# shravan-d/SculptMate

Measured on AMD Instinct MI355X. Metric: meshes/sec + ms/image, TripoSR 256^3 grid, at 1/2/4/8 MI355X, higher is better.
Workload: dtype fp32-equivalent (bf16 3-limb split, 24 bits, fp32 accumulate) density MLP / f32 tables, SiLU, marching cubes / bf16 transformer [filtered grid: an fp16 one-product pass decides the SIGN away from the level, every value marching cubes reads carries the three-limb value: mesh bit-identical to the full

## Files before the change

### sculptmate_amd/csrc/gemm.hip

```cpp
#include <stdlib.h>

#include <mutex>
#include <type_traits>

#include "common.h"

namespace sculpt {

typedef __bf16 bf16x8_t __attribute__((ext_vector_type(8)));
typedef __attribute__((address_space(3))) void *lds_ptr_t;
typedef const __attribute__((address_space(1))) void *gbl_ptr_t;

static constexpr int BM_DEFAULT = 128;
#ifndef SCULPT_GEMM_READ_AHEAD
#define SCULPT_GEMM_READ_AHEAD 1
#endif
static constexpr int BK = 64;

__device__ __forceinline__ float erf_as(float x) {
    const float ax = fabsf(x);
    const float t = __builtin_amdgcn_rcpf(fmaf(0.3275911f, ax, 1.0f));
    float p = fmaf(1.061405429f, t, -1.453152027f);
    p = fmaf(p, t, 1.421413741f);
    p = fmaf(p, t, -0.284496736f);
    p = fmaf(p, t, 0.254829592f);
    const float e = __builtin_amdgcn_exp2f(-1.44269504088896340736f * ax * ax);
    const float r = 1.0f - p * t * e;
    return copysignf(r, x);
}
__device__ __forceinline__ float gelu_erf(float x) { return 0.5f * x * (1.0f + erf_as(x * 0.70710678118654752440f)); }

__device__ __forceinline__ int lds_off(int r, int c) { return r * 128 + ((c ^ ((r >> 1) & 7)) << 4); }

struct GemmArgs {
    const uint16_t *A; int lda;
    const uint16_t *W; int ldw;
    const float *bias;
    const float *residual; int ldr;
    float *out_f32; uint16_t *out_bf16; int ldo;
    uint16_t *out_t; int ldt;
    int M, N, K;
    int n_split;
    int n_major;
    int n_store;
    int cv_H, cv_W, cv_c64, cv_dil;
    const uint16_t *cv_zero;
    const float *ln_stats; int ln_slots;
    const float *ln_colsum;
    float ln_eps;
    float *stats_out;
    int stats_ld;
    const float *zeros;
    int gm;
    int m_store;
    int stage;
    unsigned long long *stamps;
};

#ifdef SCULPT_EXPERIMENTS
unsigned long long *g_gemm_stamps = nullptr;
extern "C" void sculpt_experiment_gemm_stamps(void *p) { g_gemm_stamps = static_cast<unsigned long long *>(p); }
#endif

__device__ __forceinline__ void gemm_tile_of(const GemmArgs &g, int lin, int gx, int gy, int &nt, int &mt) {
    const int tile = xcd_tile(lin, gx * gy);
    if (g.gm > 0) {
        const int per = g.gm * gx, grp = tile / per, first = grp * g.gm, within = tile - grp * per;
        const int gsz = min(g.gm, gy - first);
        nt = within / gsz;
        mt = first + (within - nt * gsz);
    } else {
        nt = g.n_major ? tile / gy : tile % gx;
        mt = g.n_major ? tile % gy : tile / gx;
    }
}

static constexpr int LN_SLOT = 64;

template <int EPI, int BW, int NW, bool CONV = false, int BM = BM_DEFAULT, int NWR = 2, bool KS = false>
__global__ __launch_bounds__(NW * 64) void gemm_bf16_kernel(GemmArgs g) {
    static_assert(NWR == 2 || (EPI == SCULPT_EPI_NONE && !CONV), "the 4 x 2 wave grid is for the plain / residual / LayerNorm-fold form");
    static_assert(!KS || (NWR == 2 && NW == 8 && EPI == SCULPT_EPI_NONE && !CONV), "the k-split pairs are for the 8-wave plain form");
    constexpr int WT = BW * 128;
    constexpr int AT = BM * 128;
    constexpr int NSTAGE = (BW == 64 || BM == 96) ? 3 : 2;
    constexpr int DIST = NSTAGE - 1;
    constexpr int XCH = NSTAGE * (WT + AT);
    __shared__ __attribute__((aligned(16))) unsigned char smem[XCH + 2 * BM * 8];
    const int tid = threadIdx.x, lane = tid & 63;
    const int wave = __builtin_amdgcn_readfirstlane(tid >> 6);
    constexpr int NWC = NW / NWR;
    constexpr int WPW = BW / NWR;
    constexpr int TJ = BM / 16 / NWC;
    const int wr = wave / NWC, wc = wave % NWC;
    constexpr int NOUT = (EPI == SCULPT_EPI_GEGLU) ? BW / 2 : BW;
    constexpr int TI = WPW / 16;
    int nt_, mt_;
    gemm_tile_of(g, blockIdx.y * gridDim.x + blockIdx.x, gridDim.x, gridDim.y, nt_, mt_);
    const int n0 = nt_ * NOUT, m0 = mt_ * BM;
    GEMM_STAMP(g, 0);

    const int srow = lane >> 3, sslot = lane & 7;
    constexpr int WI = BW / 8 / NW;
    constexpr int AG = BM / 8, AI = (AG + NW - 1) / NW, AFULL = AG - NW * (AI - 1);
    constexpr bool UNEVEN = AG % NW != 0;
    const int acnt = (!UNEVEN || wave < AFULL) ? AI : AI - 1;
    const int abase = (!UNEVEN || wave < AFULL) ? wave * AI : AFULL * AI + (wave - AFULL) * (AI - 1);
    const uint16_t *wsrc0, *wsrc1, *wsrc2, *wsrc3;
    const uint16_t *asrc0, *asrc1, *asrc2, *asrc3;
    unsigned amask0 = 0, amask1 = 0, amask2 = 0, amask3 = 0;
    const uint16_t *zsrc = CONV ? g.cv_zero + (sslot << 3) : nullptr;
    {
        auto wrow = [&](int j) -> int {
            if (EPI == SCULPT_EPI_GEGLU) {
                const int sub = j >> 4, within = j & 15;
                return ((sub & 1) ? g.N : 0) + n0 + (sub >> 1) * 16 + within;
            }
            return n0 + j;
        };
        auto wp = [&](int q) -> const uint16_t * {
            const int r = 8 * (wave * WI + q) + srow;
            return g.W + (long)wrow(r) * g.ldw + ((sslot ^ ((r >> 1) & 7)) << 3);
        };
        auto ap = [&](int q) -> const uint16_t * {
            const int r = 8 * (abase + q) + srow;
            const int m = min(m0 + r, g.M - 1);
            return g.A + (long)m * g.lda + ((sslot ^ ((r >> 1) & 7)) << 3);
        };
        auto am = [&](int q) -> unsigned {
            if (!CONV) return 0u;
            const int r = 8 * (abase + q) + srow;
            const int m = min(m0 + r, g.M - 1);
            const int x = m % g.cv_W, y = (m / g.cv_W) % g.cv_H;
            unsigned mask = 0;
#pragma unroll
            for (int t = 0; t < 9; ++t) {
                const int yy = y + (t / 3 - 1) * g.cv_dil, xx = x + (t % 3 - 1) * g.cv_dil;
                mask |= (yy >= 0 && yy < g.cv_H && xx >= 0 && xx < g.cv_W) ? (1u << t) : 0u;
            }
            return mask;
        };
        wsrc0 = wp(0); wsrc1 = wp(1 % WI); wsrc2 = wp(2 % WI); wsrc3 = wp(3 % WI);
        asrc0 = ap(0); asrc1 = ap(1 % AI); asrc2 = ap(2 % AI); asrc3 = ap(3 % AI);
        amask0 = am(0); amask1 = am(1 % AI); amask2 = am(2 % AI); amask3 = am(3 % AI);
    }
    const int wdst = (wave * WI) * 1024, adst = abase * 1024;

#define STAGE(buf, kt)                                                                                       \
    do {                                                                                                     \
        unsigned char *wb = smem + (buf) * (WT + AT);                                                        \
        unsigned char *ab = wb + WT;                                                                         \
        const int ko = (kt) * BK;                                                                            \
        __builtin_amdgcn_global_load_lds((gbl_ptr_t)(wsrc0 + ko), (lds_ptr_t)(wb + wdst), 16, 0, 0);         \
        if (WI >= 2)                                                                                         \
            __builtin_amdgcn_global_load_lds((gbl_ptr_t)(wsrc1 + ko), (lds_ptr_t)(wb + wdst + 1024), 16, 0, 0); \
        if (WI == 4) {                                                                                       \
            __builtin_amdgcn_global_load_lds((gbl_ptr_t)(wsrc2 + ko), (lds_ptr_t)(wb + wdst + 2048), 16, 0, 0); \
            __builtin_amdgcn_global_load_lds((gbl_ptr_t)(wsrc3 + ko), (lds_ptr_t)(wb + wdst + 3072), 16, 0, 0); \
        }                                                                                                    \
        long ao = ko;                                                                                        \
        int tap = 0;                                                                                         \
        if (CONV) {                                                                                          \
            tap = (kt) / g.cv_c64;                                                                           \
            const int cc = (kt) - tap * g.cv_c64, dy = tap / 3 - 1, dx = tap - (tap / 3) * 3 - 1;            \
            ao = ((long)(dy * g.cv_dil) * g.cv_W + dx * g.cv_dil) * g.lda + cc * 64;                         \
        }                                                                                                    \
        const uint16_t *a0 = (!CONV || ((amask0 >> tap) & 1u)) ? asrc0 + ao : zsrc;                          \
        const uint16_t *a1 = (!CONV || ((amask1 >> tap) & 1u)) ? asrc1 + ao : zsrc;                          \
        __builtin_amdgcn_global_load_lds((gbl_ptr_t)a0, (lds_ptr_t)(ab + adst), 16, 0, 0);                   \
        if (AI >= 2 && (!UNEVEN || acnt >= 2))                                                               \
            __builtin_amdgcn_global_load_lds((gbl_ptr_t)a1, (lds_ptr_t)(ab + adst + 1024), 16, 0, 0);        \
        if (AI >= 3) {                                                                                       \
            const uint16_t *a2 = (!CONV || ((amask2 >> tap) & 1u)) ? asrc2 + ao : zsrc;                      \
            __builtin_amdgcn_global_load_lds((gbl_ptr_t)a2, (lds_ptr_t)(ab + adst + 2048), 16, 0, 0);        \
        }                                                                                                    \
        if (AI == 4) {                                                                                       \
            const uint16_t *a3 = (!CONV || ((amask3 >> tap) & 1u)) ? asrc3 + ao : zsrc;                      \
            __builtin_amdgcn_global_load_lds((gbl_ptr_t)a3, (lds_ptr_t)(ab + adst + 3072), 16, 0, 0);        \
        }                                                                                                    \
    } while (0)

    f32x4 acc[TI][TJ];
#pragma unroll
    for (int i = 0; i < TI; ++i)
#pragma unroll
        for (int j = 0; j < TJ; ++j) acc[i][j] = f32x4{0.f, 0.f, 0.f, 0.f};
    f32x4 acc2[KS ? 2 * TI : 1][KS ? TJ : 1];
    if (KS) {
#pragma unroll
        for (int i = 0; i < 2 * TI; ++i)
#pragma unroll
            for (int j = 0; j < TJ; ++j) acc2[KS ? i : 0][KS ? j : 0] = f32x4{0.f, 0.f, 0.f, 0.f};
    }

    const int nk = g.K / BK;
    const int fr = lane & 15, fq = lane >> 4;
    int aoff[TI], boff[TJ];
#pragma unroll
    for (int i = 0; i < TI; ++i) aoff[i] = lds_off(wr * WPW + i * 16 + fr, fq);
    int aoff2[KS ? 2 * TI : 1];
    if (KS) {
#pragma unroll
        for (int i = 0; i < 2 * TI; ++i) aoff2[KS ? i : 0] = lds_off((i / TI) * WPW + (i % TI) * 16 + fr, fq) ^ (wr << 6);
    }
#pragma unroll
    for (int j = 0; j < TJ; ++j) boff[j] = lds_off(wc * (16 * TJ) + j * 16 + fr, fq);

    constexpr int MAXU = 4;
    float2 sv[TJ][MAXU];
    const bool ln_load = g.ln_stats && wr == 0;
    if (ln_load) {
#pragma unroll
        for (int j = 0; j < TJ; ++j) {
            const int m = min(m0 + wc * (16 * TJ) + j * 16 + fr, g.M - 1);
            const float2 *sp = reinterpret_cast<const float2 *>(g.ln_stats) + m;
#pragma unroll
            for (int u = 0; u < MAXU; ++u) sv[j][u] = sp[(long)min(fq + 4 * u, g.ln_slots - 1) * g.stats_ld];
        }
    }

    constexpr int LPT = WI + AI;
    STAGE(0, 0);
    if (DIST > 1 && nk > 1) STAGE(1, 1);
    for (int kt = 0; kt < nk; ++kt) {
        const int buf = kt % NSTAGE;
        if (DIST > 1 && kt + 1 < nk && !(kt == 0 && g.ln_stats)) {
            if (!UNEVEN || acnt == AI) asm volatile("s_waitcnt vmcnt(%0)" ::"n"(LPT) : "memory");
            else asm volatile("s_waitcnt vmcnt(%0)" ::"n"(LPT - 1) : "memory");
        } else {
            asm volatile("s_waitcnt vmcnt(0)" ::: "memory");
        }
        __builtin_amdgcn_s_barrier();
#ifdef SCULPT_EXPERIMENTS
        if (kt == 0) GEMM_STAMP(g, 1);
#endif
        if (kt + DIST < nk) STAGE((kt + DIST) % NSTAGE, kt + DIST);
        const unsigned char *wb = smem + buf * (WT + AT);
        const unsigned char *ab = wb + WT;
        if constexpr (KS) {
            bf16x8_t af[2 * TI], bfr[TJ];
#pragma unroll
            for (int i = 0; i < 2 * TI; ++i) af[i] = *reinterpret_cast<const bf16x8_t *>(wb + aoff2[i]);
#pragma unroll
            for (int j = 0; j < TJ; ++j) bfr[j] = *reinterpret_cast<const bf16x8_t *>(ab + (boff[j] ^ (wr << 6)));
#pragma unroll
            for (int i = 0; i < 2 * TI; ++i)
#pragma unroll
                for (int j = 0; j < TJ; ++j)
                    acc2[i][j] = __builtin_amdgcn_mfma_f32_16x16x32_bf16(af[i], bfr[j], acc2[i][j], 0, 0, 0);
            __builtin_amdgcn_sched_group_barrier(0x100, 2 * TI + TJ, 0);
            __builtin_amdgcn_sched_group_barrier(0x8, 2 * TI * TJ, 0);
        } else if ((NW == 8 || (NW == 4 && BM == 96)) && SCULPT_GEMM_READ_AHEAD) {
            bf16x8_t af[2][TI], bfr[2][TJ];
#pragma unroll
            for (int ks = 0; ks < 2; ++ks) {
#pragma unroll
                for (int i = 0; i < TI; ++i) af[ks][i] = *reinterpret_cast<const bf16x8_t *>(wb + (aoff[i] ^ (ks << 6)));
#pragma unroll
                for (int j = 0; j < TJ; ++j) bfr[ks][j] = *reinterpret_cast<const bf16x8_t *>(ab + (boff[j] ^ (ks << 6)));
            }
#pragma unroll
            for (int ks = 0; ks < 2; ++ks)
#pragma unroll
                for (int i = 0; i < TI; ++i)
#pragma unroll
                    for (int j = 0; j < TJ; ++j)
                        acc[i][j] = __builtin_amdgcn_mfma_f32_16x16x32_bf16(af[ks][i], bfr[ks][j], acc[i][j], 0, 0, 0);
            __builtin_amdgcn_sched_group_barrier(0x100, 2 * (TI + TJ), 0);
            __builtin_amdgcn_sched_group_barrier(0x8, 2 * TI * TJ, 0);
        } else {
#pragma unroll
        for (int ks = 0; ks < 2; ++ks) {
            bf16x8_t af[TI], bfr[TJ];
#pragma unroll
            for (int i = 0; i < TI; ++i) af[i] = *reinterpret_cast<const bf16x8_t *>(wb + (aoff[i] ^ (ks << 6)));
#pragma unroll
            for (int j = 0; j < TJ; ++j) bfr[j] = *reinterpret_cast<const bf16x8_t *>(ab + (boff[j] ^ (ks << 6)));
#pragma unroll
            for (int i = 0; i < TI; ++i)
#pragma unroll
                for (int j = 0; j < TJ; ++j)
                    acc[i][j] = __builtin_amdgcn_mfma_f32_16x16x32_bf16(af[i], bfr[j], acc[i][j], 0, 0, 0);
        }
        }
    }
#undef STAGE
    if constexpr (KS) {
        asm volatile("s_waitcnt lgkmcnt(0)" ::: "memory");
        __builtin_amdgcn_s_barrier();
        f32x4 *xb = reinterpret_cast<f32x4 *>(smem);
        const int partner = (1 - wr) * NWC + wc;
        static_assert(NW * TI * TJ * 64 * 16 <= NSTAGE * (WT + AT), "the exchange fits the ring");
        if (wr == 0) {
#pragma unroll
            for (int i = 0; i < TI; ++i)
#pragma unroll
                for (int j = 0; j < TJ; ++j) xb[(wave * TI * TJ + i * TJ + j) * 64 + lane] = acc2[TI + i][j];
        } else {
#pragma unroll
            for (int i = 0; i < TI; ++i)
#pragma unroll
                for (int j = 0; j < TJ; ++j) xb[(wave * TI * TJ + i * TJ + j) * 64 + lane] = acc2[i][j];
        }
        asm volatile("s_waitcnt lgkmcnt(0)" ::: "memory");
        __builtin_amdgcn_s_barrier();
        if (wr == 0) {
#pragma unroll
            for (int i = 0; i < TI; ++i)
#pragma unroll
                for (int j = 0; j < TJ; ++j) acc[i][j] = acc2[i][j] + xb[(partner * TI * TJ + i * TJ + j) * 64 + lane];
        } else {
#pragma unroll
            for (int i = 0; i < TI; ++i)
#pragma unroll
                for (int j = 0; j < TJ; ++j) acc[i][j] = xb[(partner * TI * TJ + i * TJ + j) * 64 + lane] + acc2[TI + i][j];
        }
    }

    GEMM_STAMP(g, 2);
    float ln_mean[TJ], ln_rstd[TJ];
#pragma unroll
    for (int j = 0; j < TJ; ++j) { ln_mean[j] = 0.f; ln_rstd[j] = 1.f; }
    float2 *xch = reinterpret_cast<float2 *>(smem + XCH);
    if (g.ln_stats) {
        if (ln_load) {
            const float inv_slots = 1.0f / (float)g.ln_slots;
#pragma unroll
            for (int j = 0; j < TJ; ++j) {
                float sm = 0.f;
#pragma unroll
                for (int u = 0; u < MAXU; ++u) sm += (fq + 4 * u < g.ln_slots) ? sv[j][u].x : 0.f;
                sm += __shfl_xor(sm, 16, 64);
                sm += __shfl_xor(sm, 32, 64);
                const float mean = sm * inv_slots;
                float m2 = 0.f;
#pragma unroll
                for (int u = 0; u < MAXU; ++u) {
                    const float d = sv[j][u].x - mean;
                    m2 += (fq + 4 * u < g.ln_slots) ? fmaf((float)LN_SLOT * d, d, sv[j][u].y) : 0.f;
                }
                m2 += __shfl_xor(m2, 16, 64);
                m2 += __shfl_xor(m2, 32, 64);
                ln_mean[j] = mean;
                ln_rstd[j] = rsqrtf(m2 * inv_slots * (1.0f / LN_SLOT) + g.ln_eps);
                if (fq == 0) xch[wc * (16 * TJ) + j * 16 + fr] = make_float2(ln_mean[j], ln_rstd[j]);
            }
        }
        asm volatile("s_waitcnt lgkmcnt(0)" ::: "memory");
        __builtin_amdgcn_s_barrier();
        if (!ln_load) {
#pragma unroll
            for (int j = 0; j < TJ; ++j) {
                const float2 v = xch[wc * (16 * TJ) + j * 16 + fr];
                ln_mean[j] = v.x;
                ln_rstd[j] = v.y;
            }
        }
    }

    const float *biasp = g.bias ? g.bias : g.zeros;
    const float *csp = g.ln_stats ? g.ln_colsum : g.zeros;
    float4 b4[TI], c4[TI];
#pragma unroll
    for (int i = 0; i < TI; ++i) {
        const int wrow = (EPI == SCULPT_EPI_GEGLU) ? ((i & 1) ? g.N : 0) + n0 + (wr * (TI / 2) + (i >> 1)) * 16 + fq * 4
                                                   : n0 + wr * WPW + i * 16 + fq * 4;
        b4[i] = *reinterpret_cast<const float4 *>(biasp + wrow);
        c4[i] = *reinterpret_cast<const float4 *>(csp + wrow);
    }
    auto f4 = [](const float4 &v, int r) -> float { return r == 0 ? v.x : (r == 1 ? v.y : (r == 2 ? v.z : v.w)); };
    float4 rs[TI][TJ];
    if (EPI != SCULPT_EPI_GEGLU && g.residual) {
#pragma unroll
        for (int j = 0; j < TJ; ++j) {
            const int m = min(m0 + wc * (16 * TJ) + j * 16 + fr, g.M - 1);
#pragma unroll
            for (int i = 0; i < TI; ++i)
                rs[i][j] = *reinterpret_cast<const float4 *>(g.residual + (long)m * g.ldr + n0 + wr * WPW + i * 16 + fq * 4);
        }
    }
#pragma unroll
    for (int j = 0; j < TJ; ++j) {
        if (EPI == SCULPT_EPI_GEGLU) {
#pragma unroll
            for (int ip = 0; ip < TI / 2; ++ip)
#pragma unroll
                for (int r = 0; r < 4; ++r) {
                    const float v = ln_rstd[j] * (acc[2 * ip][j][r] - ln_mean[j] * f4(c4[2 * ip], r)) + f4(b4[2 * ip], r);
                    const float gt = ln_rstd[j] * (acc[2 * ip + 1][j][r] - ln_mean[j] * f4(c4[2 * ip + 1], r)) + f4(b4[2 * ip + 1], r);
                    acc[2 * ip][j][r] = v * gelu_erf(gt);
                }
        } else {
#pragma unroll
            for (int i = 0; i < TI; ++i)
#pragma unroll
                for (int r = 0; r < 4; ++r) {
                    float v = ln_rstd[j] * (acc[i][j][r] - ln_mean[j] * f4(c4[i], r)) + f4(b4[i], r);
                    if (EPI == SCULPT_EPI_GELU) v = gelu_erf(v);
                    if (EPI == SCULPT_EPI_RELU) v = fmaxf(v, 0.f);
                    if (g.residual) v += f4(rs[i][j], r);
                    acc[i][j][r] = v;
                }
        }
    }
    GEMM_STAMP(g, 3);
#pragma unroll
    for (int j = 0; j < TJ; ++j) {
        const int m = m0 + wc * (16 * TJ) + j * 16 + fr;
        if (m >= g.m_store) continue;
        if (EPI == SCULPT_EPI_GEGLU) {
#pragma unroll
            for (int ip = 0; ip < TI / 2; ++ip) {
                const int n = n0 + (wr * (TI / 2) + ip) * 16 + fq * 4;
                const f32x4 o = acc[2 * ip][j];
                if (g.out_bf16) {
                    uint2 pk;
                    pk.x = pack_bf16x2(o[0], o[1]);
                    pk.y = pack_bf16x2(o[2], o[3]);
                    *reinterpret_cast<uint2 *>(g.out_bf16 + (long)m * g.ldo + n) = pk;
                }
                if (g.out_f32) *reinterpret_cast<float4 *>(g.out_f32 + (long)m * g.ldo + n) = make_float4(o[0], o[1], o[2], o[3]);
            }
        } else {
#pragma unroll
            for (int i = 0; i < TI; ++i) {
                const int n = n0 + wr * WPW + i * 16 + fq * 4;
                if (n >= g.n_store) continue;
                const f32x4 o = acc[i][j];
                const bool tpart = n >= g.n_split;
                if (!tpart) {
                    if (g.out_f32) *reinterpret_cast<float4 *>(g.out_f32 + (long)m * g.ldo + n) = make_float4(o[0], o[1], o[2], o[3]);
                    if (g.out_bf16) {
                        uint2 pk;
                        pk.x = pack_bf16x2(o[0], o[1]);
                        pk.y = pack_bf16x2(o[2], o[3]);
                        *reinterpret_cast<uint2 *>(g.out_bf16 + (long)m * g.ldo + n) = pk;
                    }
                }
                if (g.out_t && (tpart || g.n_split >= g.N)) {
                    const int nt0 = tpart ? n - g.n_split : n;
#pragma unroll
                    for (int r = 0; r < 4; ++r) g.out_t[(long)(nt0 + r) * g.ldt + m] = f32_to_bf16(o[r]);
                }
            }
        }
    }
    if (EPI == SCULPT_EPI_NONE && g.stats_out) {
        constexpr int WCOLS = WPW;
        float pm[TJ], pq[TJ];
#pragma unroll
        for (int j = 0; j < TJ; ++j) {
            float sm = 0.f;
#pragma unroll
            for (int i = 0; i < TI; ++i) sm += (acc[i][j][0] + acc[i][j][1]) + (acc[i][j][2] + acc[i][j][3]);
            sm += __shfl_xor(sm, 16, 64);
            sm += __shfl_xor(sm, 32, 64);
            const float mean = sm * (1.0f / WCOLS);
            float m2 = 0.f;
#pragma unroll
            for (int i = 0; i < TI; ++i)
#pragma unroll
                for (int r = 0; r < 4; ++r) { const float d = acc[i][j][r] - mean; m2 = fmaf(d, d, m2); }
            m2 += __shfl_xor(m2, 16, 64);
            m2 += __shfl_xor(m2, 32, 64);
            pm[j] = mean;
            pq[j] = m2;
        }
        float2 *so = reinterpret_cast<float2 *>(g.stats_out);
        if (WCOLS == LN_SLOT) {
#pragma unroll
            for (int j = 0; j < TJ; ++j) {
                const int m = m0 + wc * (16 * TJ) + j * 16 + fr;
                if (fq == 0 && m < g.m_store) so[(long)((n0 + wr * WCOLS) / LN_SLOT) * g.stats_ld + m] = make_float2(pm[j], pq[j]);
            }
        } else {
            static_assert(WCOLS == LN_SLOT || 2 * WCOLS == LN_SLOT, "statistics slice = one or two waves' columns");
            if ((wr & 1) == 1 && fq == 0) {
#pragma unroll
                for (int j = 0; j < TJ; ++j) xch[(wr >> 1) * BM + wc * (16 * TJ) + j * 16 + fr] = make_float2(pm[j], pq[j]);
            }
            asm volatile("s_waitcnt lgkmcnt(0)" ::: "memory");
            __builtin_amdgcn_s_barrier();
            if ((wr & 1) == 0 && fq == 0) {
#pragma unroll
                for (int j = 0; j < TJ; ++j) {
                    const int m = m0 + wc * (16 * TJ) + j * 16 + fr;
                    const float2 o = xch[(wr >> 1) * BM + wc * (16 * TJ) + j * 16 + fr];
                    const float d = pm[j] - o.x;
                    if (m < g.m_store) so[(long)((n0 + wr * WCOLS) / LN_SLOT) * g.stats_ld + m] = make_float2(0.5f * (pm[j] + o.x), pq[j] + o.y + (0.5f * WCOLS) * d * d);
                }
            }
        }
    }
    GEMM_STAMP(g, 4);
    GEMM_STAMP_IDS(g);
}

template <int EPI, int BM, bool RES = false>
__global__ __launch_bounds__(512) void gemm256_kernel(GemmArgs g) {
    static_assert(BM == 256 || BM == 192, "activation rows per tile");
    static_assert(!RES || (BM == 192 && EPI == SCULPT_EPI_NONE), "the residual form: 192-row tiles, no activation");
    constexpr int BW = 256, NW = 8, NWC = 4, TI = 8, TJ = BM / 64, WROWS = BM / 4;
    constexpr int JB1 = TJ - 2, AU = BM / 64;
    constexpr int NU = 4 + AU;
    constexpr int WT = BW * 128, AT = BM * 128;
    constexpr int XCH = 2 * (WT + AT);
    constexpr int XBC = XCH + 2 * BM * 8;
    __shared__ __attribute__((aligned(16))) unsigned char smem[XBC + 2048];
    const int tid = threadIdx.x, lane = tid & 63;
    const int wave = __builtin_amdgcn_readfirstlane(tid >> 6);
    const int wr = wave / NWC, wc = wave % NWC;
    constexpr int NOUT = (EPI == SCULPT_EPI_GEGLU) ? BW / 2 : BW;
    int nt_, mt_;
    gemm_tile_of(g, blockIdx.y * gridDim.x + blockIdx.x, gridDim.x, gridDim.y, nt_, mt_);
    const int n0 = nt_ * NOUT, m0 = mt_ * BM;
    GEMM_STAMP(g, 0);

    const int srow = lane >> 3, sslot = lane & 7;
    unsigned woff[4], aof[4];
#pragma unroll
    for (int q = 0; q < 4; ++q) {
        const int r = 8 * (wave * 4 + q) + srow;
        const int ra = 8 * (wave * AU + (q < AU ? q : AU - 1)) + srow;
        int wrow = n0 + r;
        if (EPI == SCULPT_EPI_GEGLU) {
            const int sub = r >> 4, within = r & 15;
            wrow = ((sub & 1) ? g.N : 0) + n0 + (sub >> 1) * 16 + within;
        }
        woff[q] = ((unsigned)wrow * (unsigned)g.ldw + ((sslot ^ ((r >> 1) & 7)) << 3)) * 2u;
        aof[q] = ((unsigned)min(m0 + ra, g.M - 1) * (unsigned)g.lda + ((sslot ^ ((ra >> 1) & 7)) << 3)) * 2u;
    }
    const char *Wb = reinterpret_cast<const char *>(g.W), *Ab = reinterpret_cast<const char *>(g.A);
    const int sdst = wave * 4096, sdsta = wave * (AU * 1024);
#define G256_STAGE(buf, kt, u)                                                                                                   \
    do {                                                                                                                         \
        unsigned char *tb = smem + (buf) * (WT + AT) + ((u) >= 4 ? WT + sdsta : sdst) + ((u) & 3) * 1024;                        \
        const char *src = ((u) >= 4 ? Ab + aof[(u) & 3] : Wb + woff[(u) & 3]) + (size_t)(kt) * (BK * 2);                         \
        __builtin_amdgcn_global_load_lds((gbl_ptr_t)src, (lds_ptr_t)tb, 16, 0, 0);                                               \
    } while (0)

    const int nk = g.K / BK;
#pragma unroll
    for (int u = 0; u < NU; ++u) G256_STAGE(0, 0, u);
    if (nk > 1) {
#pragma unroll
        for (int u = 0; u < 6; ++u) G256_STAGE(1, 1, u);
    }

    const int fr = lane & 15, fq = lane >> 4;
    if (tid < 128) {
        const float *srcv = tid < 64 ? (g.bias ? g.bias : g.zeros) : (g.ln_stats ? g.ln_colsum : g.zeros);
        const int e = (tid & 63) * 4;
        const int row = EPI == SCULPT_EPI_GEGLU ? (e < 128 ? n0 + e : g.N + n0 + e - 128) : n0 + e;
        *reinterpret_cast<float4 *>(smem + XBC + (tid >> 6) * 1024 + e * 4) = *reinterpret_cast<const float4 *>(srcv + row);
    }
    float ln_mean[TJ], ln_rstd[TJ];
#pragma unroll
    for (int j = 0; j < TJ; ++j) { ln_mean[j] = 0.f; ln_rstd[j] = 1.f; }
    float2 *xch = reinterpret_cast<float2 *>(smem + XCH);
    if (g.ln_stats) {
        if (wr == 0) {
            constexpr int MAXU = 4;
            const float inv_slots = 1.0f / (float)g.ln_slots;
#pragma unroll
            for (int j = 0; j < TJ; ++j) {
                const int m = min(m0 + wc * WROWS + j * 16 + fr, g.M - 1);
                const float2 *sp = reinterpret_cast<const float2 *>(g.ln_stats) + m;
                float2 sv[MAXU];
#pragma unroll
                for (int u = 0; u < MAXU; ++u) sv[u] = sp[(long)min(fq + 4 * u, g.ln_slots - 1) * g.stats_ld];
                float sm = 0.f;
#pragma unroll
                for (int u = 0; u < MAXU; ++u) sm += (fq + 4 * u < g.ln_slots) ? sv[u].x : 0.f;
                sm += __shfl_xor(sm, 16, 64);
                sm += __shfl_xor(sm, 32, 64);
                const float mean = sm * inv_slots;
                float m2 = 0.f;
#pragma unroll
                for (int u = 0; u < MAXU; ++u) {
                    const float d = sv[u].x - mean;
                    m2 += (fq + 4 * u < g.ln_slots) ? fmaf((float)LN_SLOT * d, d, sv[u].y) : 0.f;
                }
                m2 += __shfl_xor(m2, 16, 64);
                m2 += __shfl_xor(m2, 32, 64);
                ln_mean[j] = mean;
                ln_rstd[j] = rsqrtf(m2 * inv_slots * (1.0f / LN_SLOT) + g.ln_eps);
                if (fq == 0) xch[wc * WROWS + j * 16 + fr] = make_float2(ln_mean[j], ln_rstd[j]);
            }
        }
        asm volatile("s_waitcnt lgkmcnt(0)" ::: "memory");
        __builtin_amdgcn_s_barrier();
        if (wr == 1) {
#pragma unroll
            for (int j = 0; j < TJ; ++j) {
                const float2 v = xch[wc * WROWS + j * 16 + fr];
                ln_mean[j] = v.x;
                ln_rstd[j] = v.y;
            }
        }
    }

    f32x4 acc[TI][TJ];
#pragma unroll
    for (int i = 0; i < TI; ++i)
#pragma unroll
        for (int j = 0; j < TJ; ++j) acc[i][j] = f32x4{0.f, 0.f, 0.f, 0.f};

    int aoff[4], boff[2];
#pragma unroll
    for (int i = 0; i < 4; ++i) aoff[i] = lds_off(wr * 128 + i * 16 + fr, fq);
#pragma unroll
    for (int j = 0; j < 2; ++j) boff[j] = WT + lds_off(wc * WROWS + j * 16 + fr, fq);
    bf16x8_t af[4][2], bq[4][2];
#define G256_LDA(buf, ih, i, ks) af[i][ks] = *reinterpret_cast<const bf16x8_t *>(smem + (buf) * (WT + AT) + (ih) * 8192 + (aoff[i] ^ ((ks) << 6)))
#define G256_LDB(buf, jh, j, ks) bq[2 * (jh) + (j)][ks] = *reinterpret_cast<const bf16x8_t *>(smem + (buf) * (WT + AT) + (jh) * 4096 + (boff[j] ^ ((ks) << 6)))
#define G256_MF(ih, jh, i, j, ks) \
    acc[4 * (ih) + (i)][2 * (jh) + (j)] = __builtin_amdgcn_mfma_f32_16x16x32_bf16(af[i][ks], bq[2 * (jh) + (j)][ks], acc[4 * (ih) + (i)][2 * (jh) + (j)], 0, 0, 0)
#define G256_FENCE __builtin_amdgcn_sched_barrier(0)

    if (nk > 1) asm volatile("s_waitcnt vmcnt(6)" ::: "memory");
    else asm volatile("s_waitcnt vmcnt(0)" ::: "memory");
    __builtin_amdgcn_s_barrier();
    GEMM_STAMP(g, 1);
#pragma unroll
    for (int ks = 0; ks < 2; ++ks) {
#pragma unroll
        for (int i = 0; i < 4; ++i) G256_LDA(0, 0, i, ks);
#pragma unroll
        for (int j = 0; j < 2; ++j) G256_LDB(0, 0, j, ks);
    }

    auto ktile = [&](int kt, auto more1_t, auto more2_t) __attribute__((always_inline)) {
        constexpr bool MORE1 = decltype(more1_t)::value, MORE2 = decltype(more2_t)::value;
        const int buf = kt & 1, nbuf = buf ^ 1;
#pragma unroll
        for (int ks = 0; ks < 2; ++ks)
#pragma unroll
            for (int i = 0; i < 4; ++i) {
                G256_MF(0, 0, i, 0, ks);
                G256_MF(0, 0, i, 1, ks);
                if (i < JB1) G256_LDB(buf, 1, i, ks);
                if (ks == 0 && i >= 2 && 4 + i < NU && MORE1) G256_STAGE(nbuf, kt + 1, 4 + i);
                G256_FENCE;
            }
#pragma unroll
        for (int ks = 0; ks < 2; ++ks)
#pragma unroll
            for (int i = 0; i < 4; ++i) {
                G256_MF(0, 1, i, 0, ks);
                if (JB1 == 2) G256_MF(0, 1, i, 1, ks);
                G256_LDA(buf, 1, i, ks);
                G256_FENCE;
            }
        asm volatile("s_waitcnt lgkmcnt(0)" ::: "memory");
        __builtin_amdgcn_s_barrier();
#pragma unroll
        for (int ks = 0; ks < 2; ++ks)
#pragma unroll
            for (int i = 0; i < 4; ++i) {
                G256_MF(1, 1, i, 0, ks);
                if (JB1 == 2) G256_MF(1, 1, i, 1, ks);
                if (ks == 0 && i < 3 && MORE2) G256_STAGE(buf, kt + 2, i);
                G256_FENCE;
            }
        if (MORE2) asm volatile("s_waitcnt vmcnt(3)" ::: "memory");
        else asm volatile("s_waitcnt vmcnt(0)" ::: "memory");
        __builtin_amdgcn_s_barrier();
#pragma unroll
        for (int ks = 0; ks < 2; ++ks)
#pragma unroll
            for (int i = 0; i < 4; ++i) {
                G256_MF(1, 0, i, 0, ks);
                G256_MF(1, 0, i, 1, ks);
                if (MORE1) G256_LDA(nbuf, 0, i, ks);
                if (MORE1 && i == 3) {
                    G256_LDB(nbuf, 0, 0, ks);
                    G256_LDB(nbuf, 0, 1, ks);
                }
                if (ks == 0 && i < 3 && MORE2) G256_STAGE(buf, kt + 2, 3 + i);
                G256_FENCE;
            }
    };
    {
// ... 503 lines not shown
```

Baseline: 124.5.

## Prefetch GEMM epilogue bias, colsum and residual loads inside the K loop

Splits the GEMM K loop into three modes so that the epilogue's bias/colsum and residual global loads are issued a few K-tiles before the end, behind the last stage prefetch. The vmcnt waits are adjusted to count these extra outstanding loads, which hides epilogue load latency under the final MFMA tiles. In exchange it raises register pressure by keeping the residual/bias registers live across the loop, and it relies on tricky vmcnt accounting.

```diff
diff --git a/sculptmate_amd/csrc/gemm.hip b/sculptmate_amd/csrc/gemm.hip
--- a/sculptmate_amd/csrc/gemm.hip
+++ b/sculptmate_amd/csrc/gemm.hip
@@ -14,6 +14,9 @@
 static constexpr int BM_DEFAULT = 128;
 #ifndef SCULPT_GEMM_READ_AHEAD
 #define SCULPT_GEMM_READ_AHEAD 1
+#endif
+#ifndef SCULPT_GEMM_EPI_AHEAD
+#define SCULPT_GEMM_EPI_AHEAD 1
 #endif
 static constexpr int BK = 64;
 
@@ -220,21 +223,85 @@
     }
 
     constexpr int LPT = WI + AI;
+
+    constexpr bool EPF = BW == 64, EPF_COL = EPF && BM != 64;
+    constexpr int EAHEAD = SCULPT_GEMM_EPI_AHEAD < DIST ? SCULPT_GEMM_EPI_AHEAD : DIST;
+    constexpr int EL_COL = EPF_COL ? 2 * TI : 0, EL_RES = (EPF && EPI != SCULPT_EPI_GEGLU) ? TI * TJ : 0;
+    static_assert(LPT + EL_COL + EL_RES <= 63, "vmcnt is a 6-bit counter");
+    static_assert(EAHEAD >= 1 && EAHEAD <= DIST, "every wait behind the prefetch is for a K-tile older than the epilogue loads");
+    const bool has_res = EPI != SCULPT_EPI_GEGLU && g.residual;
+    const float *biasp = g.bias ? g.bias : g.zeros;
+    const float *csp = g.ln_stats ? g.ln_colsum : g.zeros;
+    float4 b4[TI], c4[TI], rs[TI][TJ];
+    if (EPF) {
+#pragma unroll
+        for (int i = 0; i < TI; ++i) {
+            b4[i] = c4[i] = make_float4(0.f, 0.f, 0.f, 0.f);
+#pragma unroll
+            for (int j = 0; j < TJ; ++j) rs[i][j] = make_float4(0.f, 0.f, 0.f, 0.f);
+        }
+    }
+    auto column_loads = [&]() __attribute__((always_inline)) {
+#pragma unroll
+        for (int i = 0; i < TI; ++i) {
+            const int wrow = (EPI == SCULPT_EPI_GEGLU) ? ((i & 1) ? g.N : 0) + n0 + (wr * (TI / 2) + (i >> 1)) * 16 + fq * 4
+                                                       : n0 + wr * WPW + i * 16 + fq * 4;
+            b4[i] = *reinterpret_cast<const float4 *>(biasp + wrow);
+            c4[i] = *reinterpret_cast<const float4 *>(csp + wrow);
+        }
+    };
+    auto residual_loads = [&]() __attribute__((always_inline)) {
+        if (has_res) {
+#pragma unroll
+            for (int j = 0; j < TJ; ++j) {
+                const int m = min(m0 + wc * (16 * TJ) + j * 16 + fr, g.M - 1);
+#pragma unroll
+                for (int i = 0; i < TI; ++i)
+                    rs[i][j] = *reinterpret_cast<const float4 *>(g.residual + (long)m * g.ldr + n0 + wr * WPW + i * 16 + fq * 4);
+            }
+        }
+    };
+    const int pf = EPF ? max(nk - 1 - EAHEAD, 0) : nk;
+#define GEMM_VMCNT(n) asm volatile("s_waitcnt vmcnt(%0)" ::"n"(n) : "memory")
+
     STAGE(0, 0);
     if (DIST > 1 && nk > 1) STAGE(1, 1);
-    for (int kt = 0; kt < nk; ++kt) {
+    auto ktile = [&](int kt, auto mode_t) __attribute__((always_inline)) {
+        constexpr int MODE = decltype(mode_t)::value;
         const int buf = kt % NSTAGE;
-        if (DIST > 1 && kt + 1 < nk && !(kt == 0 && g.ln_stats)) {
-            if (!UNEVEN || acnt == AI) asm volatile("s_waitcnt vmcnt(%0)" ::"n"(LPT) : "memory");
-            else asm volatile("s_waitcnt vmcnt(%0)" ::"n"(LPT - 1) : "memory");
+        const bool counted = DIST > 1 && kt + 1 < nk && !(kt == 0 && g.ln_stats);
+        const bool full = !UNEVEN || acnt == AI;
+        if (MODE < 2) {
+            if (counted) {
+                if (full) GEMM_VMCNT(LPT);
+                else GEMM_VMCNT(LPT - 1);
+            } else {
+                GEMM_VMCNT(0);
+            }
+        } else if (has_res) {
+            if (counted) {
+                if (full) GEMM_VMCNT(LPT + EL_COL + EL_RES);
+                else GEMM_VMCNT(LPT - 1 + EL_COL + EL_RES);
+            } else {
+                GEMM_VMCNT(EL_COL + EL_RES);
+            }
         } else {
-            asm volatile("s_waitcnt vmcnt(0)" ::: "memory");
+            if (counted) {
+                if (full) GEMM_VMCNT(LPT + EL_COL);
+                else GEMM_VMCNT(LPT - 1 + EL_COL);
+            } else {
+                GEMM_VMCNT(EL_COL);
+            }
         }
         __builtin_amdgcn_s_barrier();
 #ifdef SCULPT_EXPERIMENTS
         if (kt == 0) GEMM_STAMP(g, 1);
 #endif
-        if (kt + DIST < nk) STAGE((kt + DIST) % NSTAGE, kt + DIST);
+        if (MODE < 2 && kt + DIST < nk) STAGE((kt + DIST) % NSTAGE, kt + DIST);
+        if (MODE == 1) {
+            if (EPF_COL) column_loads();
+            residual_loads();
+        }
         const unsigned char *wb = smem + buf * (WT + AT);
         const unsigned char *ab = wb + WT;
         if constexpr (KS) {
@@ -283,8 +350,17 @@
                     acc[i][j] = __builtin_amdgcn_mfma_f32_16x16x32_bf16(af[i], bfr[j], acc[i][j], 0, 0, 0);
         }
         }
+    };
+    {
+        int kt = 0;
+        for (; kt < pf; ++kt) ktile(kt, std::integral_constant<int, 0>{});
+        if (EPF) {
+            ktile(kt, std::integral_constant<int, 1>{});
+            for (++kt; kt < nk; ++kt) ktile(kt, std::integral_constant<int, 2>{});
+        }
     }
 #undef STAGE
+#undef GEMM_VMCNT
     if constexpr (KS) {
         asm volatile("s_waitcnt lgkmcnt(0)" ::: "memory");
         __builtin_amdgcn_s_barrier();
@@ -358,27 +434,9 @@
         }
     }
 
-    const float *biasp = g.bias ? g.bias : g.zeros;
-    const float *csp = g.ln_stats ? g.ln_colsum : g.zeros;
-    float4 b4[TI], c4[TI];
-#pragma unroll
-    for (int i = 0; i < TI; ++i) {
-        const int wrow = (EPI == SCULPT_EPI_GEGLU) ? ((i & 1) ? g.N : 0) + n0 + (wr * (TI / 2) + (i >> 1)) * 16 + fq * 4
-                                                   : n0 + wr * WPW + i * 16 + fq * 4;
-        b4[i] = *reinterpret_cast<const float4 *>(biasp + wrow);
-        c4[i] = *reinterpret_cast<const float4 *>(csp + wrow);
-    }
+    if (!EPF_COL) column_loads();
+    if (!EPF) residual_loads();
     auto f4 = [](const float4 &v, int r) -> float { return r == 0 ? v.x : (r == 1 ? v.y : (r == 2 ? v.z : v.w)); };
-    float4 rs[TI][TJ];
-    if (EPI != SCULPT_EPI_GEGLU && g.residual) {
-#pragma unroll
-        for (int j = 0; j < TJ; ++j) {
-            const int m = min(m0 + wc * (16 * TJ) + j * 16 + fr, g.M - 1);
-#pragma unroll
-            for (int i = 0; i < TI; ++i)
-                rs[i][j] = *reinterpret_cast<const float4 *>(g.residual + (long)m * g.ldr + n0 + wr * WPW + i * 16 + fq * 4);
-        }
-    }
 #pragma unroll
     for (int j = 0; j < TJ; ++j) {
         if (EPI == SCULPT_EPI_GEGLU) {
```

Measured after the change: 124.5, median of 2. Within noise of the previous version (-0.0%).
